# KyungMinJin/OTPose

Hardware: AMD Instinct MI355X
Metric: frames/sec at 384x288, 5-frame window, batch 16; heatmap max-abs delta vs ref (higher is better)
Workload: dtype f32 storage+accumulate / f16x3 split products; 1 GPU; BASELINE configs[1]: batch 16 x 5-frame x 384x288, HRNet-W48 + DCN warp + ConvVideoTransformer, fp32 forward (eval), seeded synthetic weights; clips_per_gpu=16, parallelism=dp1, outputs_finite=True

## Files before the change

### include/otpose_hip.h

```cpp
#ifndef OTPOSE_HIP_H
#define OTPOSE_HIP_H

#include <stddef.h>

#ifdef __cplusplus
extern "C" {
#endif

#define OTP_OK 0
#define OTP_ERR_BAD_ARG (-1)
#define OTP_ERR_UNSUPPORTED (-2)
#define OTP_ERR_LAUNCH (-3)
#define OTP_ERR_WORKSPACE (-4)

#define OTP_DTYPE_F32 0
#define OTP_DTYPE_F16 1
#define OTP_DTYPE_BF16 2
#define OTP_DTYPE_F64 3

#define OTP_ACT_NONE 0
#define OTP_ACT_RELU 1
#define OTP_ACT_GELU 2

int otp_version(void);
// ... 156 lines not shown
                     int B, int J, int HW, int F, void* stream);
int otp_glue_stack_n(const void* rough, const void* margin, const void* squeezed, const void* inter,
                     const void* ctx, const void* pe1, const void* pe2, void* x1, void* x2, void* prev_b,
                     int B, int J, int HW, int F, void* stream);

int otp_ln_channel(const void* x, const void* gamma, const void* beta, void* y, void* pool,
                   int B, int C, int T, float eps, void* stream);
int otp_dwconv_ln3(const void* x, const void* dwq, const void* dwk, const void* dwv,
                   const void* gq, const void* bq, const void* gk, const void* bk, const void* gv, const void* bv,
                   void* q, void* k, void* v, int B, int C, int T, int stride, float eps, void* stream);
size_t otp_chan_attn_workspace(int B, int C, int T, int n_head);
int otp_chan_attn(const void* q, const void* k, const void* v, void* out, void* workspace, size_t workspace_bytes,
                  int B, int C, int T, int n_head, float scale, void* stream);
int otp_upsample_linear(const void* x, void* out, int B, int C, int T, int f, int out_ctot, int out_coff, void* stream);

int otp_mlp_fused_supported(int C, int HID, int T);
size_t otp_mlp_fused_weight_bytes(int C, int HID);
int otp_mlp_fused_pack(const void* w1, const void* b1, const void* w2, void* packed, int C, int HID, void* stream);
int otp_mlp_fused(const void* x, const void* packed, const void* scale, const void* shift, const void* res, void* out,
                  int B, int C, int HID, int T, void* stream);
int otp_ln_mlp_fused(const void* y, const void* ln_gamma, const void* ln_beta, float ln_eps, const void* packed,
                     const void* scale, const void* shift, void* out, int B, int C, int HID, int T, void* stream);

int otp_dense_x3_supported(int C, int T);
size_t otp_dense_x3_weight_bytes(int C);
int otp_dense_x3_pack(const void* w, const void* scale, const void* shift, void* packed, int C, void* stream);
int otp_dense_x3(const void* const* x, const void* const* packed, const void* const* res, void* const* out, int nprob, int B,
                 int C, int T, void* stream);
int otp_dense_x3_pack_bf16p(const void* w, const void* scale, const void* shift, void* packed, int C, void* stream);
int otp_dense_x3_bf16p(const void* const* x, const void* const* packed, const void* const* res, void* const* out, int nprob, int B,
                 int C, int T, void* stream);
int otp_qkv_front_x3(const void* x, const void* table, const void* packed_q, const void* packed_k, const void* packed_v,
                     void* q, void* k, void* v, int B, int C, int T, float eps, void* stream);

int otp_stem_conv_x3_supported(int B, int F, int H, int W, int Cout);
size_t otp_stem_conv_x3_weight_bytes(int Cout);
int otp_stem_conv_x3_pack(const void* w, const void* scale, const void* shift, void* packed, int Cout, void* stream);
int otp_stem_conv_x3(const void* in, const void* packed, void* out, int B, int F, int H, int W, int Cout, void* stream);

int otp_pointwise_x3_supported(int Cin, int Cout, int T);
size_t otp_pointwise_x3_weight_bytes(int Cin, int Cout);
int otp_pointwise_x3_pack(const void* w, const void* scale, const void* shift, void* packed, int Cin, int Cout, void* stream);
int otp_pointwise_x3(const void* x, const void* packed, const void* res, void* out, int B, int Cin, int Cout, int T, int x_ctot,
                     int x_coff, int res_ctot, int res_coff, int out_ctot, int out_coff, int relu, void* stream);
int otp_pointwise_x3_s8_supported(int Cin, int Cout, int T);
size_t otp_pointwise_x3_s8_weight_bytes(int Cin, int Cout);
int otp_pointwise_x3_s8_pack(const void* w, const void* scale, const void* shift, void* packed, int Cin, int Cout, void* stream);
int otp_pointwise_x3_s8(const void* x, const void* packed, void* out_s8, int B, int Cin, int Cout, int T, int x_ctot, int x_coff,
                        int relu, void* stream);
int otp_pointwise_x3_s8_res(const void* x, const void* packed, const void* res, void* out_s8, int B, int Cin, int Cout, int T,
                            int x_ctot, int x_coff, int r_ctot, int r_coff, int relu, void* stream);

int otp_mlp_x3_supported(int C, int HID, int T);
size_t otp_mlp_x3_weight_bytes(int C, int HID);
int otp_mlp_x3_pack(const void* w1, const void* b1, const void* w2, void* packed, int C, int HID, void* stream);
int otp_mlp_x3(const void* x, const void* packed, const void* scale, const void* shift, const void* res, void* out, int B,
               int C, int HID, int T, void* stream);
int otp_ln_mlp_x3(const void* y, const void* ln_gamma, const void* ln_beta, float ln_eps, const void* packed,
                  const void* scale, const void* shift, void* out, int B, int C, int HID, int T, void* stream);

int otp_flow_block_supported(int C, int hidden, int T);
size_t otp_flow_front_param_floats(int C);
size_t otp_flow_back_param_floats(int C, int hidden);
int otp_flow_front(const void* x, const void* params, void* q, void* k, void* v, int B, int C, int T, float eps, void* stream);
int otp_flow_back(const void* x, const void* att, const void* params, void* out, int B, int C, int hidden, int T, float eps,
                  void* stream);
// ... 147 lines not shown
```

### otpose_amd/csrc/densex.hip

```cpp
#include "common.h"
#ifndef OTP_ENTRY
#define OTP_ENTRY(name) name
#endif

namespace {

typedef otp_x3x8 h16x8;
typedef otp_x3x2 h16x2;
typedef float f32x4 __attribute__((ext_vector_type(4)));
typedef float f32x2 __attribute__((ext_vector_type(2)));
typedef unsigned int u32x4 __attribute__((ext_vector_type(4)));

__device__ __forceinline__ void dx_split8(const float (&v)[8], h16x8& hi, h16x8& lo) {
    uint32_t h[4], l[4];
#pragma unroll
    for (int i = 0; i < 4; ++i) {
        const f32x2 a = {v[2 * i], v[2 * i + 1]};
        const uint32_t hb = __builtin_bit_cast(uint32_t, __builtin_convertvector(a, h16x2));
        const f32x2 af = otp_x3_widen(hb);
        h[i] = hb;
        l[i] = __builtin_bit_cast(uint32_t, __builtin_convertvector(a - af, h16x2));
    }
    hi = __builtin_bit_cast(h16x8, (u32x4){h[0], h[1], h[2], h[3]});
    lo = __builtin_bit_cast(h16x8, (u32x4){l[0], l[1], l[2], l[3]});
}

__device__ __forceinline__ float dx_kslot_sum(float v) {
    v += __shfl_xor(v, 16, 64);
    v += __shfl_xor(v, 32, 64);
    return v;
}

constexpr int dx_ks(int C) { return (C + 31) / 32; }
// ... 114 lines not shown
    constexpr int KS = dx_ks(C), BLKB = dx_block_bytes(C);
    __shared__ __attribute__((aligned(16))) unsigned char lds[2 * BLKB];
    const int tid = threadIdx.x, lane = tid & 63, wave = tid >> 6, kq = lane >> 4, n = lane & 15;
    const int b = blockIdx.x / tiles_per_b, tile = blockIdx.x - b * tiles_per_b;
    const int tok = tile * 128 + wave * 32 + 2 * n;
    const bool valid = tok < T;
    const size_t base = (size_t)b * C * T;
    const float* __restrict__ x = A.x[blockIdx.y];
    dx_stage<BLKB>(A.packed[blockIdx.y], lds);
    h16x8 Xh[KS][2], Xl[KS][2];
#pragma unroll
    for (int ks = 0; ks < KS; ++ks) {
        float v0[8], v1[8];
#pragma unroll
        for (int j = 0; j < 8; ++j) {
            const int c = 32 * ks + 8 * kq + j;
            const bool live = 32 * ks + 24 + j < C || c < C;
            const f32x2 v = *reinterpret_cast<const f32x2*>(x + base + (size_t)(live ? c : 0) * T + (valid ? tok : T - 2));
            v0[j] = live ? v.x : 0.f;
            v1[j] = live ? v.y : 0.f;
        }
        dx_split8(v0, Xh[ks][0], Xl[ks][0]);
        dx_split8(v1, Xh[ks][1], Xl[ks][1]);
    }
    __syncthreads();
    dx_project<C, true, H1>(Xh, Xl, A.packed[blockIdx.y], lds, A.res[blockIdx.y], A.out[blockIdx.y], base, T, tok, valid, rflag);
}

struct QxArgs {
    const unsigned char* packed[3];
    float* out[3];
};

template <int C, bool H1 = false>
__global__ __launch_bounds__(256, C <= 136 ? 3 : 1) void qkvx_front_kernel(const float* __restrict__ x, const float* __restrict__ table,
                                                            QxArgs A, int T, int tiles_per_b, float eps, unsigned* rflag) {
    constexpr int KS = dx_ks(C), BLKB = dx_block_bytes(C), TAB = 3 * C * 8;
    __shared__ __attribute__((aligned(16))) unsigned char lds[2 * BLKB];
    __shared__ __attribute__((aligned(16))) float tab[TAB];
    const int tid = threadIdx.x, lane = tid & 63, wave = tid >> 6, kq = lane >> 4, n = lane & 15;
    const int b = blockIdx.x / tiles_per_b, tile = blockIdx.x - b * tiles_per_b;
    const int tok = tile * 128 + wave * 32 + 2 * n;
    const bool valid = tok < T;
    const int tokc = valid ? tok : T - 2;
    const bool l_ok = tokc >= 1, r_ok = tokc + 2 < T;
    const size_t base = (size_t)b * C * T;
    const otp_rsrc rx = make_rsrc(x + base, (size_t)C * T * sizeof(float));
    constexpr float inv_c = 1.f / (float)C;
    const int vb0 = (8 * kq * T + tokc) * 4;
    for (int i = tid; i < TAB / 4; i += 256)
        reinterpret_cast<f32x4*>(tab)[i] = reinterpret_cast<const f32x4*>(table)[i];
    __syncthreads();

    for (int p = (int)blockIdx.y; p <= (int)blockIdx.y; ++p) {
        dx_stage<BLKB>(A.packed[p], lds);
        const float* tp = tab + p * C * 8;
        float X0[KS][8], X1[KS][8];
        float s0 = 0.f, s1 = 0.f;
#pragma unroll
        for (int ks = 0; ks < KS; ++ks) {
#pragma unroll
            for (int j = 0; j < 8; ++j) {
                const int c = 32 * ks + 8 * kq + j;
                const bool live = 32 * ks + 24 + j < C || c < C;
                const int so = (32 * ks + j) * T * 4;
                const f32x2 m = __builtin_bit_cast(f32x2, __builtin_amdgcn_raw_buffer_load_b64(rx, live ? vb0 : -16, so, 0));
                const float la = bload(rx, live ? vb0 - 4 : -16, so), ld = bload(rx, live ? vb0 + 8 : -16, so);
                const float a = l_ok ? la : 0.f, d = r_ok ? ld : 0.f;
                const f32x4 w = *reinterpret_cast<const f32x4*>(tp + (live ? c : 0) * 8);
                X0[ks][j] = live ? w[0] * a + w[1] * m.x + w[2] * m.y : 0.f;
                X1[ks][j] = live ? w[0] * m.x + w[1] * m.y + w[2] * d : 0.f;
                s0 += X0[ks][j];
                s1 += X1[ks][j];
            }
        }
        const float m0 = dx_kslot_sum(s0) * inv_c, m1 = dx_kslot_sum(s1) * inv_c;
        float v0 = 0.f, v1 = 0.f;
#pragma unroll
        for (int ks = 0; ks < KS; ++ks)
#pragma unroll
            for (int j = 0; j < 8; ++j) {
                const bool live = 32 * ks + 24 + j < C || 32 * ks + 8 * kq + j < C;
                X0[ks][j] = live ? X0[ks][j] - m0 : 0.f;
                X1[ks][j] = live ? X1[ks][j] - m1 : 0.f;
                v0 += X0[ks][j] * X0[ks][j];
                v1 += X1[ks][j] * X1[ks][j];
            }
        const float r0 = 1.f / sqrtf(dx_kslot_sum(v0) * inv_c + eps), r1 = 1.f / sqrtf(dx_kslot_sum(v1) * inv_c + eps);
        h16x8 Xh[KS][2], Xl[KS][2];
#pragma unroll
        for (int ks = 0; ks < KS; ++ks) {
#pragma unroll
            for (int j = 0; j < 8; ++j) {
                const int c = 32 * ks + 8 * kq + j;
                const bool live = 32 * ks + 24 + j < C || c < C;
                const float g = tp[(live ? c : 0) * 8 + 3], be = tp[(live ? c : 0) * 8 + 4];
                X0[ks][j] = live ? X0[ks][j] * r0 * g + be : 0.f;
                X1[ks][j] = live ? X1[ks][j] * r1 * g + be : 0.f;
            }
            dx_split8(X0[ks], Xh[ks][0], Xl[ks][0]);
            dx_split8(X1[ks], Xh[ks][1], Xl[ks][1]);
        }
        __syncthreads();
        dx_project<C, false, H1>(Xh, Xl, A.packed[p], lds, nullptr, A.out[p], base, T, tok, valid, rflag);
    }
}
// ... 34 lines not shown
        if (!a.x[i] || !a.packed[i] || !a.out[i]) return OTP_ERR_BAD_ARG;
        if ((reinterpret_cast<uintptr_t>(a.x[i]) | reinterpret_cast<uintptr_t>(a.res[i]) | reinterpret_cast<uintptr_t>(a.out[i])) & 7 ||
            reinterpret_cast<uintptr_t>(a.packed[i]) & 15)
            return OTP_ERR_BAD_ARG;
    }
    const int tiles = otp_ceil_div(T, 128);
    const dim3 grid((unsigned)(B * tiles), (unsigned)nprob);
    auto st = static_cast<hipStream_t>(stream);
    if (C == 204) {
        if (h1) hipLaunchKernelGGL((densex_cc_kernel<204, true>), grid, dim3(256), 0, st, a, T, tiles, otp_range_word());
        else hipLaunchKernelGGL((densex_cc_kernel<204, false>), grid, dim3(256), 0, st, a, T, tiles, otp_range_word());
    } else {
        if (h1) hipLaunchKernelGGL((densex_cc_kernel<136, true>), grid, dim3(256), 0, st, a, T, tiles, otp_range_word());
        else hipLaunchKernelGGL((densex_cc_kernel<136, false>), grid, dim3(256), 0, st, a, T, tiles, otp_range_word());
    }
    return otp_launch_status();
}
}

extern "C" int OTP_ENTRY(otp_dense_x3)(const void* const* x, const void* const* packed, const void* const* res, void* const* out,
                            int nprob, int B, int C, int T, void* stream) {
    return dx_dense_launch(x, packed, res, out, nprob, B, C, T, stream, false);
}

#ifndef OTP_X3_GRAD_COPY
extern "C" int otp_dense_h1(const void* const* x, const void* const* packed, const void* const* res, void* const* out, int nprob, int B,
                            int C, int T, void* stream) {
    return dx_dense_launch(x, packed, res, out, nprob, B, C, T, stream, true);
}
#endif

#ifndef OTP_X3_GRAD_COPY
namespace {
int dx_qkv_launch(const void* x, const void* table, const void* packed_q, const void* packed_k, const void* packed_v, void* q, void* k,
                  void* v, int B, int C, int T, float eps, void* stream, bool h1) {
    if (!x || !table || !packed_q || !packed_k || !packed_v || !q || !k || !v || B <= 0) return OTP_ERR_BAD_ARG;
    if (!otp_dense_x3_supported(C, T)) return OTP_ERR_UNSUPPORTED;
    if ((reinterpret_cast<uintptr_t>(x) | reinterpret_cast<uintptr_t>(q) | reinterpret_cast<uintptr_t>(k) |
         reinterpret_cast<uintptr_t>(v)) & 7 ||
        (reinterpret_cast<uintptr_t>(table) | reinterpret_cast<uintptr_t>(packed_q) | reinterpret_cast<uintptr_t>(packed_k) |
         reinterpret_cast<uintptr_t>(packed_v)) & 15)
        return OTP_ERR_BAD_ARG;
    if ((size_t)C * T * sizeof(float) >= (1ull << 31)) return OTP_ERR_UNSUPPORTED;
    QxArgs a;
    a.packed[0] = static_cast<const unsigned char*>(packed_q); a.packed[1] = static_cast<const unsigned char*>(packed_k);
    a.packed[2] = static_cast<const unsigned char*>(packed_v);
    a.out[0] = static_cast<float*>(q); a.out[1] = static_cast<float*>(k); a.out[2] = static_cast<float*>(v);
    const int tiles = otp_ceil_div(T, 128);
    const dim3 grid((unsigned)(B * tiles), 3u);
    auto st = static_cast<hipStream_t>(stream);
    auto xf = static_cast<const float*>(x), tf = static_cast<const float*>(table);
    if (C == 204) {
        if (h1) hipLaunchKernelGGL((qkvx_front_kernel<204, true>), grid, dim3(256), 0, st, xf, tf, a, T, tiles, eps, otp_range_word());
        else hipLaunchKernelGGL((qkvx_front_kernel<204, false>), grid, dim3(256), 0, st, xf, tf, a, T, tiles, eps, otp_range_word());
    } else {
        if (h1) hipLaunchKernelGGL((qkvx_front_kernel<136, true>), grid, dim3(256), 0, st, xf, tf, a, T, tiles, eps, otp_range_word());
        else hipLaunchKernelGGL((qkvx_front_kernel<136, false>), grid, dim3(256), 0, st, xf, tf, a, T, tiles, eps, otp_range_word());
    }
    return otp_launch_status();
}
}

extern "C" int otp_qkv_front_x3(const void* x, const void* table, const void* packed_q, const void* packed_k,
                                const void* packed_v, void* q, void* k, void* v, int B, int C, int T, float eps, void* stream) {
    return dx_qkv_launch(x, table, packed_q, packed_k, packed_v, q, k, v, B, C, T, eps, stream, false);
}

extern "C" int otp_qkv_front_h1(const void* x, const void* table, const void* packed_q, const void* packed_k,
                                const void* packed_v, void* q, void* k, void* v, int B, int C, int T, float eps, void* stream) {
    return dx_qkv_launch(x, table, packed_q, packed_k, packed_v, q, k, v, B, C, T, eps, stream, true);
}
#endif
```

### otpose_amd/engine.py

```python
from __future__ import annotations

import ctypes
import os
import sys
import warnings
from typing import Callable, List

import torch

from . import hip, ops
from .ops import ACT_GELU, ACT_NONE, ACT_RELU, View

BN_EPS = 1e-5


def _pair(v):
    return (int(v), int(v)) if isinstance(v, int) else (int(v[0]), int(v[1]))


class InferenceEngine:
    def __init__(self, model, batch: int, device, use_graph: bool | None = None, stream_set: int = 0, inp=None, margin=None):
        device = torch.device(device)
        if device.type != "cuda" or not torch.cuda.is_available():
            raise RuntimeError("otpose_amd.OTPose runs on an MI355X through libotpose_hip.so; "
                               f"got device '{device}' (there is no CPU or PyTorch-op fallback)")
        self.lib = hip.lib()
        self.dev = device
        self.B = batch
        self.model = model
        cfg = model.cfg
        self.J = model.num_joints
        self.F = getattr(model, "window_frames", 5)
        self.W_img, self.H_img = cfg.MODEL.IMAGE_SIZE
        self.h, self.w = model.pe_h, model.pe_w
        self.ops: List[Callable] = []
        self._aux = {}
        self._keep = []
        self._bufs = []
        self._stream = None
        if use_graph is None:
            use_graph = os.environ.get("OTPOSE_HIP_GRAPH", "1") != "0"
        self.use_graph = use_graph
        self.use_winograd = os.environ.get("OTPOSE_WINOGRAD", "1") != "0"
        self.use_x3 = os.environ.get("OTPOSE_CONV_MATH", "x3") != "f32"
        self.use_dcn_fused = self.use_x3 and os.environ.get("OTPOSE_DCN_FUSED", "1") != "0"
        self.use_s8 = self.use_x3 and os.environ.get("OTPOSE_S8", "1") != "0"
        self.use_flow_fused = os.environ.get("OTPOSE_FLOW_FUSED", "1") != "0"
        self.use_small_conv = os.environ.get("OTPOSE_SMALL_CONV", "1") != "0"
        self.use_fused_mlp = os.environ.get("OTPOSE_FUSED_MLP", "1") != "0"
        self.fuse_shortcut = os.environ.get("OTPOSE_FUSE_SHORTCUT", "1") != "0"
        self.fuse_upsample = os.environ.get("OTPOSE_FUSE_UPSAMPLE", "1") != "0"
        self.use_dense_cc = os.environ.get("OTPOSE_DENSE_CC", "1") != "0"
        self.use_qkv_front = os.environ.get("OTPOSE_QKV_FRONT", "1") != "0"
        self.use_pointx = self.use_x3 and os.environ.get("OTPOSE_POINTX", "1") != "0"
        self.multi_stream = os.environ.get("OTPOSE_STREAMS", "1") != "0"
        self.f32_tail = int(os.environ.get("OTPOSE_F32_TAIL", "0")) if self.use_x3 else 0
        self._exact = False
        self._sid = 0
        self.half_products = bool(getattr(self, "h16", False)) and self.use_x3 and os.environ.get("OTPOSE_H16_TAIL", "1") != "0"
        self.range_check = os.environ.get("OTPOSE_RANGE_CHECK", "defer")
        self._side = hip.side_streams(device, 3, 4 * stream_set) if self.multi_stream else []
        self._given = (inp, margin)
        self.graph = None
        self.param_version = self._param_version()
        with torch.no_grad():
            self._build()

    @classmethod
    def bare(cls, device, multi_stream=False):
        self = cls.__new__(cls)
        device = torch.device(device)
        if device.type != "cuda" or not torch.cuda.is_available():
            raise RuntimeError("InferenceEngine.bare needs the GPU (there is no CPU or PyTorch-op fallback)")
        env = os.environ.get
        self.lib, self.dev, self.model, self.B = hip.lib(), device, None, 0
        self.ops, self._aux, self._keep, self._bufs, self._stream = [], {}, [], [], None
        self.use_graph, self.graph = False, None
        self.use_winograd = env("OTPOSE_WINOGRAD", "1") != "0"
        self.use_x3 = env("OTPOSE_CONV_MATH", "x3") != "f32"
        self.use_dcn_fused = self.use_x3 and env("OTPOSE_DCN_FUSED", "1") != "0"
        self.use_s8 = self.use_x3 and env("OTPOSE_S8", "1") != "0"
        self.use_flow_fused = env("OTPOSE_FLOW_FUSED", "1") != "0"
        self.use_small_conv = env("OTPOSE_SMALL_CONV", "1") != "0"
        self.use_fused_mlp = env("OTPOSE_FUSED_MLP", "1") != "0"
        self.fuse_shortcut = env("OTPOSE_FUSE_SHORTCUT", "1") != "0"
        self.fuse_upsample = env("OTPOSE_FUSE_UPSAMPLE", "1") != "0"
        self.use_dense_cc = env("OTPOSE_DENSE_CC", "1") != "0"
        self.use_qkv_front = env("OTPOSE_QKV_FRONT", "1") != "0"
        self.use_pointx = self.use_x3 and env("OTPOSE_POINTX", "1") != "0"
        self.multi_stream = bool(multi_stream)
        self.f32_tail, self._exact = 0, False
        self._sid = 0
        self.half_products = False
        self.range_check = env("OTPOSE_RANGE_CHECK", "defer")
        self._side = hip.side_streams(device, 3, 0) if self.multi_stream else []
        self.inp = None
        return self

    def matches(self, x) -> bool:
        return (x.shape[0] == self.B and x.device == self.dev and tuple(x.shape[2:]) == (self.H_img, self.W_img)
                and self._param_version() == self.param_version)

    def matches_shape(self, b, c, h, w, dev) -> bool:
        return (b == self.B and dev == self.dev and (h, w) == (self.H_img, self.W_img) and c == 3 * self.F
                and self._param_version() == self.param_version)

    def _param_version(self):
        ts = getattr(self, "_tracked", None)
        if ts is None:
            ts = self._tracked = list(self.model.parameters()) + list(self.model.buffers())
        v = a = 0
        for t in ts:
            v += t._version
            a ^= t.data_ptr()
        return (len(ts), v, a)

    def new(self, *shape):
        t = torch.empty(shape, dtype=torch.float32, device=self.dev)
        rng = os.environ.get("OTPOSE_POISON")
        if rng:
            lo, hi = (int(v) for v in rng.split(":"))
# ... 602 lines not shown
                self._exact = s == 4 and mi >= len(mods) - self.f32_tail
                ys = self.hr_module(mod, ys, fork_in=not (mi > 0 and prev_cont), join_out=not cont) if mi > 0 else \
                    self.hr_module(mod, ys, fork_in=True, join_out=not cont)
                prev_cont = cont
        fl = net.final_layer
        rough = View(self.new(self.F * self.B, self.J, self.h, self.w))
        self._exact = self.f32_tail > 0
        out = self.conv(ys[0], fl.weight, rough, 1, fl.padding[0], 1, bias=fl.bias)
        self._exact = False
        return out

    def v3(self, t3):
        b, c, t = t3.shape
        return View(t3.view(b, c, 1, t))

    def tblock(self, blk, x, stride):
        B, C, T = x.shape
        To = T if stride == 1 else (T + 2 - 3) // 2 + 1
        L = self.lib
        a = blk.attn
        if self.use_flow_fused and stride == 1 and ops.flow_block_supported(blk, C, T):
            fp, bp = ops.pack_flow_front(blk, self.dev), ops.pack_flow_back(blk, self.dev)
            self._keep += [fp, bp]
            q, k, v, att, out = (self.new(B, C, T) for _ in range(5))
            self.call(L.otp_flow_front, "otp_flow_front", hip.ptr(x), hip.ptr(fp), hip.ptr(q), hip.ptr(k), hip.ptr(v),
                      B, C, T, blk.ln1.eps)
            nbytes = L.otp_chan_attn_workspace(B, C, T, a.n_head)
            ws = self.new(max(nbytes // 4, 1))
            self.call(L.otp_chan_attn, "otp_chan_attn", hip.ptr(q), hip.ptr(k), hip.ptr(v), hip.ptr(att), hip.ptr(ws),
                      nbytes, B, C, T, a.n_head, a.scale)
            self.call(L.otp_flow_back, "otp_flow_back", hip.ptr(x), hip.ptr(att), hip.ptr(bp), hip.ptr(out), B, C,
                      blk.mlp[0].out_channels, T, blk.ln2.eps)
            return out
        ln1 = self.new(B, C, T)
        skip = self.new(B, C, To) if stride > 1 else None
        p = self.dev_param
        self.call(L.otp_ln_channel, "otp_ln_channel", hip.ptr(x), hip.ptr(p(blk.ln1.weight)), hip.ptr(p(blk.ln1.bias)),
                  hip.ptr(ln1), hip.ptr(skip), B, C, T, blk.ln1.eps)
        q, k, v = self.new(B, C, To), self.new(B, C, To), self.new(B, C, To)
        dx3 = self.use_dense_cc and self.use_x3 and ops.dense_x3_supported(C, To)
        dense = dx3 or (self.use_dense_cc and ops.dense_cc_supported(C, To))
        if dense:
            packs = [ops.pack_dense_cc(m.weight.to(self.dev), None, m.bias.to(self.dev), x3=dx3)
                     for m in (a.query, a.key, a.value)]
        if dense and stride == 1 and self.use_qkv_front:
            table = ops.pack_qkv_table(*[p(t) for t in (a.query_conv.weight, a.key_conv.weight, a.value_conv.weight,
                                                         a.query_norm.weight, a.query_norm.bias, a.key_norm.weight,
                                                         a.key_norm.bias, a.value_norm.weight, a.value_norm.bias)])
            self._keep += [table, *packs]
            self.call((L.otp_qkv_front_h1 if self.half_products else L.otp_qkv_front_x3) if dx3 else L.otp_qkv_front, "otp_qkv_front",
                      hip.ptr(ln1), hip.ptr(table),
                      *[hip.ptr(t) for t in packs],
                      hip.ptr(q), hip.ptr(k), hip.ptr(v), B, C, T, a.query_norm.eps)
        else:
            qn, kn, vn = self.new(B, C, To), self.new(B, C, To), self.new(B, C, To)
            self.call(L.otp_dwconv_ln3, "otp_dwconv_ln3", hip.ptr(ln1), hip.ptr(p(a.query_conv.weight)),
                      hip.ptr(p(a.key_conv.weight)), hip.ptr(p(a.value_conv.weight)),
                      hip.ptr(p(a.query_norm.weight)), hip.ptr(p(a.query_norm.bias)),
                      hip.ptr(p(a.key_norm.weight)), hip.ptr(p(a.key_norm.bias)),
                      hip.ptr(p(a.value_norm.weight)), hip.ptr(p(a.value_norm.bias)),
                      hip.ptr(qn), hip.ptr(kn), hip.ptr(vn), B, C, T, stride, a.query_norm.eps)
            if dense:
                self.dense((qn, kn, vn), packs, None, (q, k, v), B, C, To)
            else:
                self.conv(self.v3(qn), a.query.weight, self.v3(q), bias=a.query.bias)
                self.conv(self.v3(kn), a.key.weight, self.v3(k), bias=a.key.bias)
                self.conv(self.v3(vn), a.value.weight, self.v3(v), bias=a.value.bias)
        att = self.new(B, C, To)
        nbytes = L.otp_chan_attn_workspace(B, C, To, a.n_head)
        ws = self.new(max(nbytes // 4, 1))
        self.call(L.otp_chan_attn, "otp_chan_attn", hip.ptr(q), hip.ptr(k), hip.ptr(v), hip.ptr(att), hip.ptr(ws),
                  nbytes, B, C, To, a.n_head, a.scale)
        sa = blk.drop_path_attn.scale.detach().reshape(-1)
        y = self.new(B, C, To)
        if dense:
            sad = sa.to(self.dev, torch.float32)
            pk = ops.pack_dense_cc(a.proj.weight.to(self.dev), sad, a.proj.bias.detach().to(self.dev) * sad,
                                   x3=self.use_x3 and ops.dense_x3_supported(C, To))
            self.dense((att,), [pk], (skip if stride > 1 else x,), (y,), B, C, To)
        else:
            self.conv(self.v3(att), a.proj.weight, self.v3(y), scale=sa,
                      shift=a.proj.bias.detach() * sa.to(a.proj.bias.device), res=self.v3(skip if stride > 1 else x))
        sm = blk.drop_path_mlp.scale.detach().reshape(-1)
        out = self.new(B, C, To)
        hid = blk.mlp[0].out_channels
        if self.use_fused_mlp and self.use_x3 and ops.mlp_x3_supported(C, hid, To):
# ... 263 lines not shown
```

### otpose_amd/hip.py

```python
from __future__ import annotations

import ctypes
import os
import threading
from ctypes import c_float, c_int, c_size_t, c_void_p

_HERE = os.path.dirname(os.path.abspath(__file__))
LIB_PATH = os.environ.get("OTPOSE_HIP_LIB") or os.path.join(_HERE, "csrc", "libotpose_hip.so")
_lib = None
_tls = threading.local()

OTP_OK = 0
_ERRORS = {
    -1: "OTP_ERR_BAD_ARG (null pointer or non-positive dimension)",
    -2: "OTP_ERR_UNSUPPORTED (shape / dtype / stride combination not implemented)",
    -3: "OTP_ERR_LAUNCH (HIP launch error)",
    -4: "OTP_ERR_WORKSPACE (workspace too small)",
}


class ConvDesc(ctypes.Structure):
    _fields_ = [(n, c_int) for n in (
        "N", "Cin", "H", "W", "Cout", "kh", "kw", "stride", "pad", "dil",
        "in_ctot", "in_coff", "in2_ctot", "in2_coff", "out_ctot", "out_coff",
# ... 106 lines not shown
    "otp_qkv_front_table_bytes": (c_size_t, [c_int]),
    "otp_qkv_front_pack_table": (c_int, [c_void_p] * 10 + [c_int, c_void_p]),
    "otp_qkv_front": (c_int, [c_void_p] * 8 + [c_int] * 3 + [c_float, c_void_p]),
    "otp_mlp_fused_supported": (c_int, [c_int] * 3),
    "otp_mlp_fused_weight_bytes": (c_size_t, [c_int] * 2),
    "otp_mlp_fused_pack": (c_int, [c_void_p] * 4 + [c_int] * 2 + [c_void_p]),
    "otp_mlp_fused": (c_int, [c_void_p] * 6 + [c_int] * 4 + [c_void_p]),
    "otp_ln_mlp_fused": (c_int, [c_void_p] * 3 + [c_float] + [c_void_p] * 4 + [c_int] * 4 + [c_void_p]),
    "otp_dcn_fused_supported": (c_int, [c_int] * 5),
    "otp_dcn_fused_weight_bytes": (c_size_t, [c_int] * 2),
    "otp_dcn_fused_pack": (c_int, [c_void_p] * 5 + [c_int, c_int, c_void_p]),
    "otp_dcn_fused_workspace": (c_size_t, [c_int] * 3),
    "otp_dcn_fused_forward": (c_int, [c_void_p] * 5 + [c_size_t] + [c_int] * 5 + [ctypes.POINTER(c_int), c_int, c_float, c_void_p]),
    "otp_dense_x3_supported": (c_int, [c_int] * 2),
    "otp_dense_x3_weight_bytes": (c_size_t, [c_int]),
    "otp_dense_x3_pack": (c_int, [c_void_p] * 4 + [c_int, c_void_p]),
    "otp_dense_x3": (c_int, [ctypes.POINTER(c_void_p)] * 4 + [c_int] * 4 + [c_void_p]),
    "otp_dense_x3_pack_bf16p": (c_int, [c_void_p] * 4 + [c_int, c_void_p]),
    "otp_dense_x3_bf16p": (c_int, [ctypes.POINTER(c_void_p)] * 4 + [c_int] * 4 + [c_void_p]),
    "otp_stem_conv_x3_supported": (c_int, [c_int] * 5),
    "otp_stem_conv_x3_weight_bytes": (c_size_t, [c_int]),
    "otp_stem_conv_x3_pack": (c_int, [c_void_p] * 4 + [c_int, c_void_p]),
    "otp_stem_conv_x3": (c_int, [c_void_p] * 3 + [c_int] * 5 + [c_void_p]),
    "otp_pointwise_x3_supported": (c_int, [c_int] * 3),
    "otp_pointwise_x3_weight_bytes": (c_size_t, [c_int] * 2),
    "otp_pointwise_x3_pack": (c_int, [c_void_p] * 4 + [c_int, c_int, c_void_p]),
    "otp_pointwise_x3": (c_int, [c_void_p] * 4 + [c_int] * 11 + [c_void_p]),
    "otp_pointwise_x3_s8_supported": (c_int, [c_int] * 3),
    "otp_pointwise_x3_s8_weight_bytes": (c_size_t, [c_int] * 2),
    "otp_pointwise_x3_s8_pack": (c_int, [c_void_p] * 4 + [c_int, c_int, c_void_p]),
    "otp_pointwise_x3_s8": (c_int, [c_void_p] * 3 + [c_int] * 7 + [c_void_p]),
    "otp_pointwise_x3_s8_res": (c_int, [c_void_p] * 4 + [c_int] * 9 + [c_void_p]),
    "otp_qkv_front_x3": (c_int, [c_void_p] * 8 + [c_int] * 3 + [c_float, c_void_p]),
    "otp_mlp_x3_supported": (c_int, [c_int] * 3),
    "otp_mlp_x3_weight_bytes": (c_size_t, [c_int] * 2),
    "otp_mlp_x3_pack": (c_int, [c_void_p] * 4 + [c_int] * 2 + [c_void_p]),
    "otp_mlp_x3": (c_int, [c_void_p] * 6 + [c_int] * 4 + [c_void_p]),
    "otp_flow_block_supported": (c_int, [c_int] * 3),
    "otp_flow_front_param_floats": (c_size_t, [c_int]),
    "otp_flow_back_param_floats": (c_size_t, [c_int, c_int]),
    "otp_flow_front": (c_int, [c_void_p] * 5 + [c_int] * 3 + [c_float, c_void_p]),
    "otp_flow_back": (c_int, [c_void_p] * 4 + [c_int] * 4 + [c_float, c_void_p]),
    "otp_ln_mlp_x3": (c_int, [c_void_p] * 3 + [c_float] + [c_void_p] * 4 + [c_int] * 4 + [c_void_p]),
    "otp_chan_attn": (c_int, [c_void_p] * 4 + [c_void_p, c_size_t] + [c_int] * 4 + [c_float, c_void_p]),
    "otp_chan_attn_splits": (c_int, [c_int, c_int]),
    "otp_chan_attn_scores": (c_int, [c_void_p] * 3 + [c_int] * 3 + [c_void_p]),
    "otp_chan_attn_set_split": (c_int, [c_int]),
    "otp_chan_attn_apply": (c_int, [c_void_p] * 3 + [c_int] * 3 + [c_void_p]),
    "otp_chan_attn_scores_bf16p": (c_int, [c_void_p] * 3 + [c_int] * 3 + [c_void_p]),
    "otp_chan_attn_apply_bf16p": (c_int, [c_void_p] * 3 + [c_int] * 3 + [c_void_p]),
    "otp_transpose_scale": (c_int, [c_void_p, c_void_p, c_int, c_int, c_int, c_float, c_void_p]),
    "otp_softmax_backward": (c_int, [c_void_p] * 5 + [c_int] * 3 + [c_void_p]),
    "otp_ln_channel_backward": (c_int, [c_void_p] * 5 + [c_int] * 3 + [c_float, c_void_p]),
    "otp_ln_channel_backward_workspace": (c_size_t, [c_int] * 3),
    "otp_ln_channel_backward_params": (c_int, [c_void_p] * 6 + [c_void_p, c_size_t] + [c_int] * 3 + [c_float, c_void_p]),
    "otp_dwconv3_forward": (c_int, [c_void_p] * 3 + [c_int] * 4 + [c_void_p]),
    "otp_dwconv3_backward": (c_int, [c_void_p] * 5 + [c_int] * 4 + [c_void_p]),
    "otp_gelu_forward": (c_int, [c_void_p, c_void_p, c_size_t, c_void_p]),
    "otp_gelu_backward": (c_int, [c_void_p] * 3 + [c_size_t, c_void_p]),
    "otp_maxpool3s2_forward": (c_int, [c_void_p, c_void_p, c_int, c_int, c_void_p]),
    "otp_maxpool3s2_backward": (c_int, [c_void_p] * 3 + [c_int, c_int, c_void_p]),
    "otp_upsample_linear_backward": (c_int, [c_void_p, c_void_p] + [c_int] * 6 + [c_void_p]),
    "otp_upsample_linear": (c_int, [c_void_p, c_void_p] + [c_int] * 6 + [c_void_p]),
    "otp_upsample_add": (c_int, [c_void_p] * 3 + [c_int] * 12 + [c_void_p]),
    "otp_upsample_add_multi": (c_int, [ctypes.POINTER(c_void_p), ctypes.POINTER(c_int), c_int, c_void_p, c_void_p] + [c_int] * 9 + [c_void_p]),
    "otp_upsample_add_backward": (c_int, [c_void_p] * 4 + [c_int] * 4 + [c_void_p]),
# ... 117 lines not shown
```

Baseline: 3127 frames/s.

## Fuse transformer block LayerNorm into QKV front kernel

Adds an LN1 variant of the QKV front kernel that reads the raw block input and computes per-token channel mean and rstd in registers. Neighbouring-token values for the depthwise temporal conv are exchanged via DPP, and halo tokens at tile edges get their stats through shared memory. This removes the separate otp_ln_channel launch and the write and re-read of the ln1 tensor. In exchange it adds an extra reduction pass and more register pressure in the front kernel, and the stats are recomputed in each of the three q/k/v blocks.

```diff
diff --git a/include/otpose_hip.h b/include/otpose_hip.h
--- a/include/otpose_hip.h
+++ b/include/otpose_hip.h
@@ -212,6 +212,12 @@
                  int C, int T, void* stream);
 int otp_qkv_front_x3(const void* x, const void* table, const void* packed_q, const void* packed_k, const void* packed_v,
                      void* q, void* k, void* v, int B, int C, int T, float eps, void* stream);
+int otp_qkv_front_ln_x3(const void* x, const void* ln_gamma, const void* ln_beta, float ln_eps, const void* table, const void* packed_q,
+                        const void* packed_k, const void* packed_v, void* q, void* k, void* v, int B, int C, int T, float eps,
+                        void* stream);
+int otp_qkv_front_ln_h1(const void* x, const void* ln_gamma, const void* ln_beta, float ln_eps, const void* table, const void* packed_q,
+                        const void* packed_k, const void* packed_v, void* q, void* k, void* v, int B, int C, int T, float eps,
+                        void* stream);
 
 int otp_stem_conv_x3_supported(int B, int F, int H, int W, int Cout);
 size_t otp_stem_conv_x3_weight_bytes(int Cout);
diff --git a/otpose_amd/csrc/densex.hip b/otpose_amd/csrc/densex.hip
--- a/otpose_amd/csrc/densex.hip
+++ b/otpose_amd/csrc/densex.hip
@@ -1,4 +1,5 @@
 #include "common.h"
+#include <type_traits>
 #ifndef OTP_ENTRY
 #define OTP_ENTRY(name) name
 #endif
@@ -179,15 +180,18 @@
     float* out[3];
 };
 
-template <int C, bool H1 = false>
+template <int C, bool H1 = false, bool LN1 = false>
 __global__ __launch_bounds__(256, C <= 136 ? 3 : 1) void qkvx_front_kernel(const float* __restrict__ x, const float* __restrict__ table,
-                                                            QxArgs A, int T, int tiles_per_b, float eps, unsigned* rflag) {
+                                                            QxArgs A, int T, int tiles_per_b, float eps, unsigned* rflag,
+                                                            const float* __restrict__ g1, const float* __restrict__ b1, float eps1) {
     constexpr int KS = dx_ks(C), BLKB = dx_block_bytes(C), TAB = 3 * C * 8;
     __shared__ __attribute__((aligned(16))) unsigned char lds[2 * BLKB];
     __shared__ __attribute__((aligned(16))) float tab[TAB];
+    __shared__ f32x2 lnp[LN1 ? C : 1];
+    __shared__ f32x2 st[LN1 ? 130 : 1];
     const int tid = threadIdx.x, lane = tid & 63, wave = tid >> 6, kq = lane >> 4, n = lane & 15;
     const int b = blockIdx.x / tiles_per_b, tile = blockIdx.x - b * tiles_per_b;
-    const int tok = tile * 128 + wave * 32 + 2 * n;
+    const int t0 = tile * 128, tok = t0 + wave * 32 + 2 * n;
     const bool valid = tok < T;
     const int tokc = valid ? tok : T - 2;
     const bool l_ok = tokc >= 1, r_ok = tokc + 2 < T;
@@ -197,6 +201,8 @@
     const int vb0 = (8 * kq * T + tokc) * 4;
     for (int i = tid; i < TAB / 4; i += 256)
         reinterpret_cast<f32x4*>(tab)[i] = reinterpret_cast<const f32x4*>(table)[i];
+    if constexpr (LN1)
+        for (int i = tid; i < C; i += 256) lnp[i] = (f32x2){g1[i], b1[i]};
     __syncthreads();
 
     for (int p = (int)blockIdx.y; p <= (int)blockIdx.y; ++p) {
@@ -204,21 +210,101 @@
         const float* tp = tab + p * C * 8;
         float X0[KS][8], X1[KS][8];
         float s0 = 0.f, s1 = 0.f;
-#pragma unroll
-        for (int ks = 0; ks < KS; ++ks) {
-#pragma unroll
-            for (int j = 0; j < 8; ++j) {
-                const int c = 32 * ks + 8 * kq + j;
-                const bool live = 32 * ks + 24 + j < C || c < C;
-                const int so = (32 * ks + j) * T * 4;
-                const f32x2 m = __builtin_bit_cast(f32x2, __builtin_amdgcn_raw_buffer_load_b64(rx, live ? vb0 : -16, so, 0));
-                const float la = bload(rx, live ? vb0 - 4 : -16, so), ld = bload(rx, live ? vb0 + 8 : -16, so);
-                const float a = l_ok ? la : 0.f, d = r_ok ? ld : 0.f;
-                const f32x4 w = *reinterpret_cast<const f32x4*>(tp + (live ? c : 0) * 8);
-                X0[ks][j] = live ? w[0] * a + w[1] * m.x + w[2] * m.y : 0.f;
-                X1[ks][j] = live ? w[0] * m.x + w[1] * m.y + w[2] * d : 0.f;
-                s0 += X0[ks][j];
-                s1 += X1[ks][j];
+        if constexpr (LN1) {
+            float E[KS][8];
+            const int ve = n == 0 ? vb0 - 4 : vb0 + 8;
+            const bool edge = n == 0 || n == 15;
+            constexpr int HN = (C + 63) / 64;
+            const int th = wave == 0 ? t0 - 1 : t0 + 128;
+            const bool hok = (wave == 0 || wave == 3) && th >= 0 && th < T;
+            float h[HN];
+#pragma unroll
+            for (int i = 0; i < HN; ++i) {
+                const int c = lane + 64 * i;
+                h[i] = bload(rx, (hok && c < C) ? (c * T + th) * 4 : -16, 0);
+            }
+#pragma unroll
+            for (int ks = 0; ks < KS; ++ks)
+#pragma unroll
+                for (int j = 0; j < 8; ++j) {
+                    const bool live = 32 * ks + 24 + j < C || 32 * ks + 8 * kq + j < C;
+                    const int so = (32 * ks + j) * T * 4;
+                    const f32x2 m = __builtin_bit_cast(f32x2, __builtin_amdgcn_raw_buffer_load_b64(rx, live ? vb0 : -16, so, 0));
+                    E[ks][j] = bload(rx, live && edge ? ve : -16, so);
+                    X0[ks][j] = live ? m.x : 0.f;
+                    X1[ks][j] = live ? m.y : 0.f;
+                    s0 += X0[ks][j];
+                    s1 += X1[ks][j];
+                }
+            const float mu0 = dx_kslot_sum(s0) * inv_c, mu1 = dx_kslot_sum(s1) * inv_c;
+            s0 = s1 = 0.f;
+            float q0 = 0.f, q1 = 0.f;
+#pragma unroll
+            for (int ks = 0; ks < KS; ++ks)
+#pragma unroll
+                for (int j = 0; j < 8; ++j) {
+                    const bool live = 32 * ks + 24 + j < C || 32 * ks + 8 * kq + j < C;
+                    X0[ks][j] = live ? X0[ks][j] - mu0 : 0.f;
+                    X1[ks][j] = live ? X1[ks][j] - mu1 : 0.f;
+                    q0 += X0[ks][j] * X0[ks][j];
+                    q1 += X1[ks][j] * X1[ks][j];
+                }
+            const float rs0 = 1.f / sqrtf(dx_kslot_sum(q0) * inv_c + eps1), rs1 = 1.f / sqrtf(dx_kslot_sum(q1) * inv_c + eps1);
+            if (kq == 0) {
+                st[tok - t0 + 1] = (f32x2){mu0, rs0};
+                st[tok - t0 + 2] = (f32x2){mu1, rs1};
+            }
+            if (wave == 0 || wave == 3) {
+                float hs = 0.f;
+#pragma unroll
+                for (int i = 0; i < HN; ++i) hs += h[i];
+                const float hm = wave_sum(hs) * inv_c;
+                float hq = 0.f;
+#pragma unroll
+                for (int i = 0; i < HN; ++i) {
+                    h[i] = lane + 64 * i < C ? h[i] - hm : 0.f;
+                    hq += h[i] * h[i];
+                }
+                const float hr = 1.f / sqrtf(wave_sum(hq) * inv_c + eps1);
+                if (lane == 0) st[wave == 0 ? 0 : 129] = (f32x2){hm, hok ? hr : 0.f};
+            }
+            __syncthreads();
+            const f32x2 se = st[n == 0 ? tokc - t0 : tokc - t0 + 3];
+#pragma unroll
+            for (int ks = 0; ks < KS; ++ks) {
+#pragma unroll
+                for (int j = 0; j < 8; ++j) {
+                    const int c = 32 * ks + 8 * kq + j;
+                    const bool live = 32 * ks + 24 + j < C || c < C;
+                    const f32x2 gb = lnp[live ? c : 0];
+                    const float m0 = X0[ks][j] * rs0 * gb.x + gb.y, m1 = X1[ks][j] * rs1 * gb.x + gb.y;
+                    const int e = __builtin_bit_cast(int, (E[ks][j] - se.x) * se.y * gb.x + gb.y);
+                    const float a = __builtin_bit_cast(float, __builtin_amdgcn_update_dpp(e, __builtin_bit_cast(int, m1), 0x111, 0xF, 0xF, false));
+                    const float d = __builtin_bit_cast(float, __builtin_amdgcn_update_dpp(e, __builtin_bit_cast(int, m0), 0x101, 0xF, 0xF, false));
+                    const f32x4 w = *reinterpret_cast<const f32x4*>(tp + (live ? c : 0) * 8);
+                    X0[ks][j] = live ? w[0] * (l_ok ? a : 0.f) + w[1] * m0 + w[2] * m1 : 0.f;
+                    X1[ks][j] = live ? w[0] * m0 + w[1] * m1 + w[2] * (r_ok ? d : 0.f) : 0.f;
+                    s0 += X0[ks][j];
+                    s1 += X1[ks][j];
+                }
+            }
+        } else {
+#pragma unroll
+            for (int ks = 0; ks < KS; ++ks) {
+#pragma unroll
+                for (int j = 0; j < 8; ++j) {
+                    const int c = 32 * ks + 8 * kq + j;
+                    const bool live = 32 * ks + 24 + j < C || c < C;
+                    const int so = (32 * ks + j) * T * 4;
+                    const f32x2 m = __builtin_bit_cast(f32x2, __builtin_amdgcn_raw_buffer_load_b64(rx, live ? vb0 : -16, so, 0));
+                    const float la = bload(rx, live ? vb0 - 4 : -16, so), ld = bload(rx, live ? vb0 + 8 : -16, so);
+                    const float a = l_ok ? la : 0.f, d = r_ok ? ld : 0.f;
+                    const f32x4 w = *reinterpret_cast<const f32x4*>(tp + (live ? c : 0) * 8);
+                    X0[ks][j] = live ? w[0] * a + w[1] * m.x + w[2] * m.y : 0.f;
+                    X1[ks][j] = live ? w[0] * m.x + w[1] * m.y + w[2] * d : 0.f;
+                    s0 += X0[ks][j];
+                    s1 += X1[ks][j];
+                }
             }
         }
         const float m0 = dx_kslot_sum(s0) * inv_c, m1 = dx_kslot_sum(s1) * inv_c;
@@ -319,9 +405,17 @@
 
 #ifndef OTP_X3_GRAD_COPY
 namespace {
-int dx_qkv_launch(const void* x, const void* table, const void* packed_q, const void* packed_k, const void* packed_v, void* q, void* k,
-                  void* v, int B, int C, int T, float eps, void* stream, bool h1) {
+template <int C, bool H1, bool LN1>
+void dx_qkv_kernel(dim3 grid, hipStream_t st, const float* x, const float* table, const QxArgs& a, int T, int tiles, float eps,
+                   const float* g1, const float* b1, float eps1) {
+    hipLaunchKernelGGL((qkvx_front_kernel<C, H1, LN1>), grid, dim3(256), 0, st, x, table, a, T, tiles, eps, otp_range_word(), g1, b1,
+                       eps1);
+}
+
+int dx_qkv_launch(const void* x, const void* const* ln1, float eps1, const void* table, const void* packed_q, const void* packed_k,
+                  const void* packed_v, void* q, void* k, void* v, int B, int C, int T, float eps, void* stream, bool h1) {
     if (!x || !table || !packed_q || !packed_k || !packed_v || !q || !k || !v || B <= 0) return OTP_ERR_BAD_ARG;
+    if (ln1 && (!ln1[0] || !ln1[1])) return OTP_ERR_BAD_ARG;
     if (!otp_dense_x3_supported(C, T)) return OTP_ERR_UNSUPPORTED;
     if ((reinterpret_cast<uintptr_t>(x) | reinterpret_cast<uintptr_t>(q) | reinterpret_cast<uintptr_t>(k) |
          reinterpret_cast<uintptr_t>(v)) & 7 ||
@@ -337,24 +431,44 @@
     const dim3 grid((unsigned)(B * tiles), 3u);
     auto st = static_cast<hipStream_t>(stream);
     auto xf = static_cast<const float*>(x), tf = static_cast<const float*>(table);
-    if (C == 204) {
-        if (h1) hipLaunchKernelGGL((qkvx_front_kernel<204, true>), grid, dim3(256), 0, st, xf, tf, a, T, tiles, eps, otp_range_word());
-        else hipLaunchKernelGGL((qkvx_front_kernel<204, false>), grid, dim3(256), 0, st, xf, tf, a, T, tiles, eps, otp_range_word());
-    } else {
-        if (h1) hipLaunchKernelGGL((qkvx_front_kernel<136, true>), grid, dim3(256), 0, st, xf, tf, a, T, tiles, eps, otp_range_word());
-        else hipLaunchKernelGGL((qkvx_front_kernel<136, false>), grid, dim3(256), 0, st, xf, tf, a, T, tiles, eps, otp_range_word());
-    }
+    auto g1 = ln1 ? static_cast<const float*>(ln1[0]) : nullptr, b1 = ln1 ? static_cast<const float*>(ln1[1]) : nullptr;
+    auto go = [&](auto c_) {
+        constexpr int CC = decltype(c_)::value;
+        if (ln1) {
+            if (h1) dx_qkv_kernel<CC, true, true>(grid, st, xf, tf, a, T, tiles, eps, g1, b1, eps1);
+            else dx_qkv_kernel<CC, false, true>(grid, st, xf, tf, a, T, tiles, eps, g1, b1, eps1);
+        } else {
+            if (h1) dx_qkv_kernel<CC, true, false>(grid, st, xf, tf, a, T, tiles, eps, nullptr, nullptr, 0.f);
+            else dx_qkv_kernel<CC, false, false>(grid, st, xf, tf, a, T, tiles, eps, nullptr, nullptr, 0.f);
+        }
+    };
+    if (C == 204) go(std::integral_constant<int, 204>());
+    else go(std::integral_constant<int, 136>());
     return otp_launch_status();
 }
 }
 
 extern "C" int otp_qkv_front_x3(const void* x, const void* table, const void* packed_q, const void* packed_k,
                                 const void* packed_v, void* q, void* k, void* v, int B, int C, int T, float eps, void* stream) {
-    return dx_qkv_launch(x, table, packed_q, packed_k, packed_v, q, k, v, B, C, T, eps, stream, false);
+    return dx_qkv_launch(x, nullptr, 0.f, table, packed_q, packed_k, packed_v, q, k, v, B, C, T, eps, stream, false);
 }
 
 extern "C" int otp_qkv_front_h1(const void* x, const void* table, const void* packed_q, const void* packed_k,
                                 const void* packed_v, void* q, void* k, void* v, int B, int C, int T, float eps, void* stream) {
-    return dx_qkv_launch(x, table, packed_q, packed_k, packed_v, q, k, v, B, C, T, eps, stream, true);
+    return dx_qkv_launch(x, nullptr, 0.f, table, packed_q, packed_k, packed_v, q, k, v, B, C, T, eps, stream, true);
+}
+
+extern "C" int otp_qkv_front_ln_x3(const void* x, const void* ln_gamma, const void* ln_beta, float ln_eps, const void* table,
+                                   const void* packed_q, const void* packed_k, const void* packed_v, void* q, void* k, void* v, int B,
+                                   int C, int T, float eps, void* stream) {
+    const void* ln1[2] = {ln_gamma, ln_beta};
+    return dx_qkv_launch(x, ln1, ln_eps, table, packed_q, packed_k, packed_v, q, k, v, B, C, T, eps, stream, false);
+}
+
+extern "C" int otp_qkv_front_ln_h1(const void* x, const void* ln_gamma, const void* ln_beta, float ln_eps, const void* table,
+                                   const void* packed_q, const void* packed_k, const void* packed_v, void* q, void* k, void* v, int B,
+                                   int C, int T, float eps, void* stream) {
+    const void* ln1[2] = {ln_gamma, ln_beta};
+    return dx_qkv_launch(x, ln1, ln_eps, table, packed_q, packed_k, packed_v, q, k, v, B, C, T, eps, stream, true);
 }
 #endif
diff --git a/otpose_amd/engine.py b/otpose_amd/engine.py
--- a/otpose_amd/engine.py
+++ b/otpose_amd/engine.py
@@ -52,6 +52,7 @@
         self.fuse_upsample = os.environ.get("OTPOSE_FUSE_UPSAMPLE", "1") != "0"
         self.use_dense_cc = os.environ.get("OTPOSE_DENSE_CC", "1") != "0"
         self.use_qkv_front = os.environ.get("OTPOSE_QKV_FRONT", "1") != "0"
+        self.tblock_fused = os.environ.get("OTPOSE_TBLOCK_FUSED", "1") != "0"
         self.use_pointx = self.use_x3 and os.environ.get("OTPOSE_POINTX", "1") != "0"
         self.multi_stream = os.environ.get("OTPOSE_STREAMS", "1") != "0"
         self.f32_tail = int(os.environ.get("OTPOSE_F32_TAIL", "0")) if self.use_x3 else 0
@@ -87,6 +88,7 @@
         self.fuse_upsample = env("OTPOSE_FUSE_UPSAMPLE", "1") != "0"
         self.use_dense_cc = env("OTPOSE_DENSE_CC", "1") != "0"
         self.use_qkv_front = env("OTPOSE_QKV_FRONT", "1") != "0"
+        self.tblock_fused = env("OTPOSE_TBLOCK_FUSED", "1") != "0"
         self.use_pointx = self.use_x3 and env("OTPOSE_POINTX", "1") != "0"
         self.multi_stream = bool(multi_stream)
         self.f32_tail, self._exact = 0, False
@@ -755,26 +757,35 @@
             self.call(L.otp_flow_back, "otp_flow_back", hip.ptr(x), hip.ptr(att), hip.ptr(bp), hip.ptr(out), B, C,
                       blk.mlp[0].out_channels, T, blk.ln2.eps)
             return out
-        ln1 = self.new(B, C, T)
-        skip = self.new(B, C, To) if stride > 1 else None
         p = self.dev_param
-        self.call(L.otp_ln_channel, "otp_ln_channel", hip.ptr(x), hip.ptr(p(blk.ln1.weight)), hip.ptr(p(blk.ln1.bias)),
-                  hip.ptr(ln1), hip.ptr(skip), B, C, T, blk.ln1.eps)
-        q, k, v = self.new(B, C, To), self.new(B, C, To), self.new(B, C, To)
         dx3 = self.use_dense_cc and self.use_x3 and ops.dense_x3_supported(C, To)
         dense = dx3 or (self.use_dense_cc and ops.dense_cc_supported(C, To))
+        front = dense and stride == 1 and self.use_qkv_front
+        ln_in_front = front and dx3 and self.tblock_fused
+        skip = self.new(B, C, To) if stride > 1 else None
+        if not ln_in_front:
+            ln1 = self.new(B, C, T)
+            self.call(L.otp_ln_channel, "otp_ln_channel", hip.ptr(x), hip.ptr(p(blk.ln1.weight)), hip.ptr(p(blk.ln1.bias)),
+                      hip.ptr(ln1), hip.ptr(skip), B, C, T, blk.ln1.eps)
+        q, k, v = self.new(B, C, To), self.new(B, C, To), self.new(B, C, To)
         if dense:
             packs = [ops.pack_dense_cc(m.weight.to(self.dev), None, m.bias.to(self.dev), x3=dx3)
                      for m in (a.query, a.key, a.value)]
-        if dense and stride == 1 and self.use_qkv_front:
+        if front:
             table = ops.pack_qkv_table(*[p(t) for t in (a.query_conv.weight, a.key_conv.weight, a.value_conv.weight,
                                                          a.query_norm.weight, a.query_norm.bias, a.key_norm.weight,
                                                          a.key_norm.bias, a.value_norm.weight, a.value_norm.bias)])
             self._keep += [table, *packs]
-            self.call((L.otp_qkv_front_h1 if self.half_products else L.otp_qkv_front_x3) if dx3 else L.otp_qkv_front, "otp_qkv_front",
-                      hip.ptr(ln1), hip.ptr(table),
-                      *[hip.ptr(t) for t in packs],
-                      hip.ptr(q), hip.ptr(k), hip.ptr(v), B, C, T, a.query_norm.eps)
+            if ln_in_front:
+                self.call(L.otp_qkv_front_ln_h1 if self.half_products else L.otp_qkv_front_ln_x3, "otp_qkv_front_ln",
+                          hip.ptr(x), hip.ptr(p(blk.ln1.weight)), hip.ptr(p(blk.ln1.bias)), blk.ln1.eps, hip.ptr(table),
+                          *[hip.ptr(t) for t in packs],
+                          hip.ptr(q), hip.ptr(k), hip.ptr(v), B, C, T, a.query_norm.eps)
+            else:
+                self.call((L.otp_qkv_front_h1 if self.half_products else L.otp_qkv_front_x3) if dx3 else L.otp_qkv_front,
+                          "otp_qkv_front", hip.ptr(ln1), hip.ptr(table),
+                          *[hip.ptr(t) for t in packs],
+                          hip.ptr(q), hip.ptr(k), hip.ptr(v), B, C, T, a.query_norm.eps)
         else:
             qn, kn, vn = self.new(B, C, To), self.new(B, C, To), self.new(B, C, To)
             self.call(L.otp_dwconv_ln3, "otp_dwconv_ln3", hip.ptr(ln1), hip.ptr(p(a.query_conv.weight)),
diff --git a/otpose_amd/hip.py b/otpose_amd/hip.py
--- a/otpose_amd/hip.py
+++ b/otpose_amd/hip.py
@@ -162,6 +162,8 @@
     "otp_pointwise_x3_s8": (c_int, [c_void_p] * 3 + [c_int] * 7 + [c_void_p]),
     "otp_pointwise_x3_s8_res": (c_int, [c_void_p] * 4 + [c_int] * 9 + [c_void_p]),
     "otp_qkv_front_x3": (c_int, [c_void_p] * 8 + [c_int] * 3 + [c_float, c_void_p]),
+    "otp_qkv_front_ln_x3": (c_int, [c_void_p] * 3 + [c_float] + [c_void_p] * 7 + [c_int] * 3 + [c_float, c_void_p]),
+    "otp_qkv_front_ln_h1": (c_int, [c_void_p] * 3 + [c_float] + [c_void_p] * 7 + [c_int] * 3 + [c_float, c_void_p]),
     "otp_mlp_x3_supported": (c_int, [c_int] * 3),
     "otp_mlp_x3_weight_bytes": (c_size_t, [c_int] * 2),
     "otp_mlp_x3_pack": (c_int, [c_void_p] * 4 + [c_int] * 2 + [c_void_p]),
```

Result: no change. 3154 frames/s, median of 6 (+0.8%).
